# codyd51/gypsum

Measured on AMD Instinct MI355X. Metric: iq_msamples_per_s_32sat_acquire_plus_track, higher is better.
Workload: dtype f32; 1 GPU; cfg3 8.184Msps x128 streams/GPU: 32-sat acquire (13 scans/step) + 12-ch E-P-L track 1000ms/step; iq=resident in HBM (host-fed: legs.h2d), streams_per_gpu=128, satellites_searched=32, scene=SURVEY d2: a*N=41, sigma=6a (lock unreachable; lock-regime legs: *_lock), parallelism=streams sharded over 1 GPU(s), one ncclAllGather/step (gyp_allgather_dev)

## Files before the change

gypsum_amd/csrc/kernels_dll_exact.hpp:

```cpp
#pragma once
#include "kernels_track_block.hpp"

namespace gyp {

struct DllExactParams {
    const cf* iq;
    int64_t stream_stride;
    int32_t n_ms, ms_begin, ms_end;
    const double* start_time;
    const ChanState* states;
    int32_t n_chan;
    const SpecIn* spec;
    double* disc_out;
    const float* chipf;
    double inv_fs;
    const int32_t* only_if;
    const int32_t* from_sub;
    SubLayout sub;
    const int32_t* trk_round;
};

__device__ __forceinline__ double2 horner64(double2 acc, double2 w, double2 x) {
    return make_double2(fma(acc.x, w.x, fma(-acc.y, w.y, x.x)), fma(acc.x, w.y, fma(acc.y, w.x, x.y)));
}
__device__ __forceinline__ double2 cvt64(cf x) { return make_double2((double)x.x, (double)x.y); }
__device__ __forceinline__ double2 cvt64(double2 x) { return x; }
struct ExactChips { float cm1, c0, cp1; };
__device__ __forceinline__ ExactChips exact_window_chips(const float* chipf, int m, int q) {
    int j = m - q;
    j = j < 0 ? j + kChips : j;
    j = j < 0 ? j + kChips : j;
    const float* cp = chipf + j + kChips;
    return ExactChips{cp[-1], cp[0], cp[1]};
}
#pragma clang diagnostic push
#pragma clang diagnostic ignored "-Walign-mismatch"
typedef float4 __attribute__((aligned(8))) float4_a8;
__device__ __forceinline__ float4 load_pair_a8(const cf* src, int pair = 0) { return reinterpret_cast<const float4_a8*>(src)[pair]; }
#pragma clang diagnostic pop
template <int K, bool EDGE>
__device__ __forceinline__ ExactChips exact_window_load(const cf* __restrict__ block, int m, int r, int q, const float* __restrict__ chipf, cf (&x)[K]) {
    constexpr int N = K * kChips;
    const int n0 = K * m + r;
    if constexpr (EDGE) {
#pragma unroll
        for (int i = 0; i < K; ++i) {
            const int n = n0 + i;
            const cf v = block[min(max(n, 0), N - 1)];
            const bool in = n >= 0 && n < N;
            x[i] = make_float2(in ? v.x : 0.f, in ? v.y : 0.f);
        }
    } else {
        const cf* src = block + n0;
#pragma unroll
        for (int i = 0; i + 1 < K; i += 2) {
            const float4 v = load_pair_a8(src + i);
            x[i] = make_float2(v.x, v.y);
            x[i + 1] = make_float2(v.z, v.w);
        }
        if (K & 1) x[K - 1] = src[K - 1];
    }
    return exact_window_chips(chipf, m, q);
}
template <int K, typename S>
__device__ __forceinline__ void exact_window_fold(const S (&x)[K], const ExactChips& c, double2 rho, double2 step, double2& sp, double2& se, double2& sl) {
    const double dj = (double)c.c0, gl = (double)(c.cm1 - c.c0), ge = (double)(c.c0 - c.cp1);
    double2 h = cvt64(x[K - 1]);
#pragma unroll
    for (int i = K - 2; i >= 0; --i) h = horner64(h, rho, cvt64(x[i]));
    const double2 xe = cvt64(x[K - 1]), xl = cvt64(x[0]);
    sp = horner64(sp, step, make_double2(dj * h.x, dj * h.y));
    se = horner64(se, step, make_double2(ge * xe.x, ge * xe.y));
    sl = horner64(sl, step, make_double2(gl * xl.x, gl * xl.y));
}
template <int K, bool EDGE>
__device__ __forceinline__ void exact_window(const cf* __restrict__ block, int m, int r, int q, const float* __restrict__ chipf,
                                             double2 rho, double2 step, double2& sp, double2& se, double2& sl) {
    cf x[K];
    const ExactChips c = exact_window_load<K, EDGE>(block, m, r, q, chipf, x);
    exact_window_fold<K>(x, c, rho, step, sp, se, sl);
}
template <int K>
__device__ __forceinline__ double2 cpow_km1(double2 w) {
    double2 r = make_double2(1.0, 0.0);
#pragma unroll
    for (int i = 0; i < K - 1; ++i) r = cmul64(r, w);
    return r;
}
struct ExactUnit {
    double du, u0;
    int q, r;
    const float* chipf;
};
template <int K>
__device__ __forceinline__ ExactUnit exact_unit(const DllExactParams& p, const SpecIn& in, int sat, int ms) {
    ExactUnit u;
    u.chipf = p.chipf + (sat - 1) * 2048;
    u.du = in.doppler * p.inv_fs;
    u.u0 = carrier_cycles(in.doppler, p.start_time[ms], in.carrier_phase);
    const int sN = __builtin_amdgcn_readfirstlane(mod_n(in.code_phase, K * kChips));
    u.q = sN / K; u.r = sN % K;
    return u;
}
template <int K>
__device__ __forceinline__ void exact_unit_store(double2 sp, double2 se, double2 sl, const ExactUnit& u, int lane, int n_anchor, double* out) {
    const double2 rho_a = carrier64(u.du);
    const double2 anchor = carrier64(u.u0 + u.du * (double)n_anchor);
    const double2 pp = cmul64(sp, anchor), ee = cmul64(cmul64(se, cpow_km1<K>(rho_a)), anchor), ll = cmul64(sl, anchor);
    double acc[6] = {pp.x, pp.y, ee.x, ee.y, ll.x, ll.y};
#pragma unroll
    for (int v = 0; v < 6; ++v) acc[v] = wave_sum_last(acc[v]);
    if (lane == 63) *out = dll_discriminator_exact(acc);
}
__device__ __forceinline__ bool exact_unit_decode(const DllExactParams& p, int u, int& ch, int& ms) {
    if (!unit_decode(p, u, ch, ms)) return false;
    if (p.only_if && !p.only_if[ch]) return false;
    if (p.from_sub && ms < p.sub.begin(p.from_sub[ch])) return false;
    return true;
}
template <int K>
__global__ __launch_bounds__(256, 4) void dll_exact_wave_kernel(DllExactParams p) {
    static_assert(K <= 8, "a window's samples in registers");
    constexpr int N = K * kChips;
    const int lane = threadIdx.x & 63;
    const int wave = __builtin_amdgcn_readfirstlane((int)(threadIdx.x >> 6));
    const int n_units = p.n_chan * unit_span(p);
    const int n_groups = (n_units + 3) >> 2;
    for (int g = blockIdx.x; g < n_groups; g += gridDim.x) {
        const int u = ((n_groups & 7) ? g : xcd_contiguous(g, n_groups)) * 4 + wave;
        if (u >= n_units) continue;
        int ch, ms;
        if (!exact_unit_decode(p, u, ch, ms)) continue;
        const int64_t at = (int64_t)ch * p.n_ms + ms;
        const SpecIn in = p.spec[at];
        if (in.key == kSpecKeyLost) continue;
        const ChanState* st = p.states + ch;
        const int sat = __builtin_amdgcn_readfirstlane(st->sat_id), stream = __builtin_amdgcn_readfirstlane(st->stream);
        const cf* block = p.iq + (int64_t)stream * p.stream_stride + (int64_t)ms * N;
        const ExactUnit x = exact_unit<K>(p, in, sat, ms);
        double2 sp = make_double2(0.0, 0.0), se = sp, sl = sp;
        const double2 rho = carrier64(x.du), step = carrier64(x.du * (double)(K * 64));
        exact_window<K, true>(block, lane + 64 * 15 - 1, x.r, x.q, x.chipf, rho, step, sp, se, sl);
#pragma unroll 2
        for (int c = 14; c >= 1; --c) exact_window<K, false>(block, lane + 64 * c - 1, x.r, x.q, x.chipf, rho, step, sp, se, sl);
        exact_window<K, true>(block, lane - 1, x.r, x.q, x.chipf, rho, step, sp, se, sl);
        exact_unit_store<K>(sp, se, sl, x, lane, K * (lane - 1) + x.r, p.disc_out + at);
    }
}
constexpr int kExactSharedConsumers = 12;
constexpr int kExactSharedProducers = 4;
constexpr int kExactSharedThreads = 64 * (kExactSharedConsumers + kExactSharedProducers);
constexpr int kExactGroupMaxChan = 16384;
struct ExactGroup {
    int32_t stream, n;
    int32_t ch[kExactSharedConsumers];
    int32_t pad[2];
};
static_assert(sizeof(ExactGroup) == 64, "ExactGroup");
template <int K>
constexpr int exact_shared_lds_units() { return (K * kChips + 2 * K) / K * (K + 1); }
template <int K>
constexpr size_t exact_shared_lds_bytes() { return (size_t)exact_shared_lds_units<K>() * sizeof(double2); }

__global__ __launch_bounds__(256) void exact_group_kernel(const ChanState* __restrict__ states, int32_t n_chan, ExactGroup* __restrict__ groups,
                                                          int32_t* __restrict__ n_groups) {
    __shared__ int32_t s_stream[kExactGroupMaxChan];
    for (int i = threadIdx.x; i < n_chan; i += blockDim.x) s_stream[i] = states[i].stream;
    __syncthreads();
    const int c = blockIdx.x * blockDim.x + threadIdx.x;
    if (c >= n_chan) return;
    const int s = s_stream[c];
    int before = 0;
    for (int i = 0; i < c; ++i) before += s_stream[i] == s ? 1 : 0;
    if (before % kExactSharedConsumers) return;
    ExactGroup g;
    g.stream = s; g.n = 1; g.ch[0] = c; g.pad[0] = g.pad[1] = 0;
#pragma unroll
    for (int k = 1; k < kExactSharedConsumers; ++k) g.ch[k] = -1;
    for (int i = c + 1; i < n_chan && g.n < kExactSharedConsumers; ++i) {
        if (s_stream[i] != s) continue;
#pragma unroll
        for (int k = 1; k < kExactSharedConsumers; ++k)
            if (k == g.n) g.ch[k] = i;
        ++g.n;
    }
    groups[atomicAdd(n_groups, 1)] = g;
}

struct DllExactSharedParams {
    DllExactParams x;
    const ExactGroup* groups;
    const int32_t* n_groups;
};
template <int K>
__global__ __launch_bounds__(kExactSharedThreads) void dll_exact_shared_kernel(DllExactSharedParams ps) {
    static_assert(K <= 8, "a window's samples in registers");
    constexpr int N = K * kChips;
    static_assert(K % 2 == 0, "the producers fetch sample pairs");
    constexpr int PT = 64 * kExactSharedProducers;
    constexpr int PAIRS = N / 2;
    constexpr int LOADS = (PAIRS + PT - 1) / PT;
    extern __shared__ double2 s_x[];
    const DllExactParams& p = ps.x;
    const int lane = threadIdx.x & 63;
    const int wave = __builtin_amdgcn_readfirstlane((int)(threadIdx.x >> 6));
    const int span = p.ms_end - p.ms_begin;
    const int64_t n_items = (int64_t)__builtin_amdgcn_readfirstlane(ps.n_groups[0]) * span;
    const int64_t lo = n_items * blockIdx.x / gridDim.x, hi = n_items * (blockIdx.x + 1) / gridDim.x;
    if (lo >= hi) return;
    if (threadIdx.x < 2 * K) {
        const int np = threadIdx.x < K ? (int)threadIdx.x : N + (int)threadIdx.x;
        s_x[np + np / K] = make_double2(0.0, 0.0);
    }
    if (wave >= kExactSharedConsumers) {
        const int pt = lane + 64 * (wave - kExactSharedConsumers);
        float4 hold[LOADS];
        auto request = [&](int64_t item) {
            const int g = (int)(item / span), ms = p.ms_begin + (int)(item % span);
            const int stream = __builtin_amdgcn_readfirstlane(ps.groups[g].stream);
            const cf* block = p.iq + (int64_t)stream * p.stream_stride + (int64_t)ms * N;
#pragma unroll
            for (int j = 0; j < LOADS; ++j) {
                const int t = pt + PT * j;
                if (PT * j + PT <= PAIRS) hold[j] = load_pair_a8(block, t);
                else hold[j] = t < PAIRS ? load_pair_a8(block, t) : make_float4(0.f, 0.f, 0.f, 0.f);
            }
        };
        request(lo);
        for (int64_t item = lo; item < hi; ++item) {
#pragma unroll
            for (int j = 0; j < LOADS; ++j) {
                const int t = pt + PT * j, np = 2 * t + K;
                if (PT * j + PT <= PAIRS || t < PAIRS) {
                    s_x[np + np / K] = make_double2((double)hold[j].x, (double)hold[j].y);
                    s_x[np + np / K + 1] = make_double2((double)hold[j].z, (double)hold[j].w);
                }
            }
            __syncthreads();
            if (item + 1 < hi) request(item + 1);
            __syncthreads();
        }
        return;
    }
    const double2* win0 = s_x + (K + 1) * lane;
    for (int64_t item = lo; item < hi; ++item) {
        __syncthreads();
        const int g = (int)(item / span), ms = p.ms_begin + (int)(item % span);
        const ExactGroup* grp = ps.groups + g;
        const int ch = wave < __builtin_amdgcn_readfirstlane(grp->n) ? __builtin_amdgcn_readfirstlane(grp->ch[wave]) : -1;
        if (ch >= 0) {
            const int64_t at = (int64_t)ch * p.n_ms + ms;
            const SpecIn in = p.spec[at];
            if (in.key != kSpecKeyLost) {
                const ExactUnit u = exact_unit<K>(p, in, __builtin_amdgcn_readfirstlane(p.states[ch].sat_id), ms);
                int off[K];
#pragma unroll
                for (int i = 0; i < K; ++i) off[i] = u.r + i + (u.r + i >= K ? 1 : 0);
                double2 sp = make_double2(0.0, 0.0), se = sp, sl = sp;
                const double2 rho = carrier64(u.du), step = carrier64(u.du * (double)(K * 64));
#pragma unroll 2
                for (int c = 15; c >= 0; --c) {
                    const double2* w = win0 + (K + 1) * 64 * c;
                    double2 x[K];
#pragma unroll
                    for (int i = 0; i < K; ++i) x[i] = w[off[i]];
                    exact_window_fold<K>(x, exact_window_chips(u.chipf, lane + 64 * c - 1, u.q), rho, step, sp, se, sl);
                }
                exact_unit_store<K>(sp, se, sl, u, lane, K * (lane - 1) + u.r, p.disc_out + at);
            }
        }
        __syncthreads();
    }
}
template <int K, int T, int NV, bool PAIRS, bool GUARD, typename ParamsT, typename UseT>
__device__ __forceinline__ void workgroup_exact_sums(const cf* block, const ParamsT& p, const SpecIn& in, int ms, int lag,
                                                     const float* chipf, int tid, double (*part)[6], UseT use) {
    static_assert(!PAIRS || T == 256, "four wavefronts");
    const double du = in.doppler * p.inv_fs;
    const double u0 = carrier_cycles(in.doppler, p.start_time[ms], in.carrier_phase);
    double acc[6];
    exact_epl_generic<K, T>(block, u0, du, lag, chipf, tid, acc);
#pragma unroll
    for (int v = 0; v < NV; ++v) acc[v] = wave_sum_last(acc[v]);
    if (GUARD) __syncthreads();
    if ((tid & 63) == 63) {
#pragma unroll
        for (int v = 0; v < NV; ++v) part[tid >> 6][v] = acc[v];
    }
    __syncthreads();
    if (tid == 0) {
        double ex[NV];
#pragma unroll
        for (int v = 0; v < NV; ++v) {
            if (PAIRS) {
                ex[v] = (part[0][v] + part[1][v]) + (part[2][v] + part[3][v]);
            } else {
                double t = part[0][v];
#pragma unroll
                for (int w = 1; w < T / 64; ++w) t += part[w][v];
                ex[v] = t;
            }
        }
        use(ex);
    }
}
template <int K>
__global__ __launch_bounds__(256) void dll_exact_block_kernel(DllExactParams p) {
    constexpr int N = K * kChips;
    __shared__ double part[4][6];
    const int tid = threadIdx.x;
    const int n_units = p.n_chan * unit_span(p);
    for (int v = blockIdx.x; v < n_units; v += gridDim.x) {
        int ch, ms;
        if (!exact_unit_decode(p, (n_units & 7) ? v : xcd_contiguous(v, n_units), ch, ms)) continue;
        const int64_t at = (int64_t)ch * p.n_ms + ms;
        const SpecIn in = p.spec[at];
        if (in.key == kSpecKeyLost) continue;
        const ChanState* st = p.states + ch;
        const cf* block = p.iq + (int64_t)st->stream * p.stream_stride + (int64_t)ms * N;
        workgroup_exact_sums<K, 256, 6, true, true>(block, p, in, ms, mod_n(in.code_phase, N), p.chipf + (st->sat_id - 1) * 2048, tid, part,
                                                    [&](const double (&ex)[6]) { p.disc_out[at] = dll_discriminator_exact(ex); });
    }
}

struct DllScanParams {
    const cf* iq;
    int64_t stream_stride;
    int32_t n_ms, ms_begin, ms_end;
    const double* start_time;
    ChanState* states;
    const ChanState* ckpt;
    int32_t n_chan;
    const SpecIn* spec;
    const double* disc;
    gyp_track_rec* rec_out;
    DllExact* exact;
    const int32_t* bad;
    int32_t only_bad;
    const int32_t* from_sub;
    SubLayout sub;
    DllExact* hist_out;
    const float* chipf;
    double inv_fs, dll_gain, dll_modulus, n_samples;
    int32_t first, final;
    int32_t* prof_delta;
    int32_t prof_from, prof_depth;
    float symbol_tau;
    const int32_t* trk_round;
    DllExact* hist;
};
constexpr int kScanThreads = 256;
constexpr int kScanChunk = 512;
constexpr int kSpecKeyRepaired = -3;
__device__ __forceinline__ void scan_stage_code(float* s_chipf, const float* chipf, int tid) {
    for (int k = tid; k < 2048; k += kScanThreads) s_chipf[k] = chipf[k];
    __syncthreads();
}
template <int K>
__global__ __launch_bounds__(kScanThreads) void dll_scan_kernel(DllScanParams p) {
    constexpr int N = K * kChips;
    __shared__ double s_disc[kScanChunk];
    __shared__ int s_cpin[kScanChunk];
    __shared__ int s_cpout[kScanChunk];
    __shared__ int s_key[kScanChunk];
    __shared__ double part[kScanThreads / 64][6];
    __shared__ float s_chipf[2048];
    __shared__ double s_a;
    __shared__ int s_s, s_pos, s_repairs;
    __shared__ int s_nund;
    __shared__ short s_und[kScanChunk];
    bool have_code = false;
    const int ch = blockIdx.x, tid = threadIdx.x;
    if (ch >= p.n_chan) return;
    if (p.bad && (p.bad[ch] != 0) != (p.only_bad != 0)) return;
    const ChanState* st = p.states + ch;
    int range_lo = p.ms_begin, range_hi = p.ms_end, sub_here = -1;
    if (p.trk_round) {
        sub_here = p.trk_round[ch];
        if (sub_here < 0) return;
        range_lo = p.sub.begin(sub_here);
        range_hi = p.sub.end(sub_here, p.n_ms);
    }
    if (tid == 0) {
        if (p.trk_round) {
            if (sub_here == 0) { s_a = p.ckpt[ch].dll_phase; s_s = p.ckpt[ch].code_phase; s_repairs = 0; }
            else { const DllExact x = p.hist[(size_t)sub_here * p.n_chan + ch]; s_a = x.dll; s_s = x.code_phase; s_repairs = x.repairs; }
        } else if (p.first && p.ckpt) { s_a = p.ckpt[ch].dll_phase; s_s = p.ckpt[ch].code_phase; s_repairs = 0; }
        else { const DllExact x = p.exact[ch]; s_a = x.dll; s_s = x.code_phase; s_repairs = p.first ? 0 : x.repairs; }
    }
    const float* chipf = p.chipf + (st->sat_id - 1) * 2048;
    const cf* stream = p.iq + (int64_t)st->stream * p.stream_stride;
    const int64_t row = (int64_t)ch * p.n_ms;
    const int ms_first = (p.only_bad && p.from_sub) ? max(p.ms_begin, p.sub.begin(min(p.from_sub[ch], p.sub.sub_of(p.n_ms - 1)))) : range_lo;
    for (int c0 = ms_first; c0 < range_hi; c0 += kScanChunk) {
        const int len = min(kScanChunk, range_hi - c0);
        for (int i = tid; i < len; i += kScanThreads) {
            const SpecIn* in = p.spec + row + c0 + i;
            const int key = in->key;
            s_key[i] = key;
            s_cpin[i] = in->code_phase;
            s_disc[i] = key == kSpecKeyLost ? 0.0 : p.disc[row + c0 + i];
        }
        if (tid == 0) { s_pos = 0; s_nund = 0; }
        __syncthreads();
        if (p.rec_out) {
            for (int i = tid; i < len; i += kScanThreads) {
                const gyp_track_rec* r = p.rec_out + row + c0 + i;
                const float pr = r->peak_re, pi = r->peak_im;
                if (s_key[i] != kSpecKeyLost && r->status != 2 && fabsf(pr) <= p.symbol_tau * __builtin_amdgcn_sqrtf(fmaf(pr, pr, pi * pi)))
                    s_und[atomicAdd(&s_nund, 1)] = (short)i;
            }
            __syncthreads();
            const int n_und = s_nund;
            for (int u = 0; u < n_und; ++u) {
                const int ms = c0 + s_und[u];
                const SpecIn in = p.spec[row + ms];
                if (!have_code) { scan_stage_code(s_chipf, chipf, tid); have_code = true; }
                int lag = mod_n(in.code_phase, N) + p.rec_out[row + ms].peak_offset;
                lag = lag >= N ? lag - N : lag;
                workgroup_exact_sums<K, kScanThreads, 1, false, false>(
                    stream + (int64_t)ms * N, p, in, ms, lag, s_chipf, tid, part,
                    [&](const double (&re)[1]) { p.rec_out[row + ms].pseudosymbol = re[0] > 0.0 ? 1 : (re[0] < 0.0 ? -1 : 0); });
                __syncthreads();
            }
        }
        while (true) {
            if (tid < 64) {
                double a = s_a;
                int s = s_s, i = __builtin_amdgcn_readfirstlane(s_pos);
                bool stop = false;
                int key_n = 0, cp_n = 0;
                double d_n = 0.0;
                if (i < len) { key_n = s_key[i]; cp_n = s_cpin[i]; d_n = s_disc[i]; }
                while (i < len && !stop) {
                    const int key = key_n, cp = cp_n;
                    const double d = d_n;
                    if (i + 1 < len) { key_n = s_key[i + 1]; cp_n = s_cpin[i + 1]; d_n = s_disc[i + 1]; }
                    const double dll = __dadd_rn(a, __dmul_rn(d, p.dll_gain));
                    const double whole = trunc(dll);
                    const int usual = (int)(key != kSpecKeyLost) & ((int)(key == kSpecKeyRepaired) | (int)(s == cp)) &
                                      (int)(fabs(whole) < 2147483648.0) & (int)(dll > -p.dll_modulus) & (int)(dll < 2.0 * p.dll_modulus);
                    if (__builtin_amdgcn_readfirstlane(usual)) {
                        double r = dll >= p.dll_modulus ? dll - p.dll_modulus : dll;
                        r += (r != 0.0 && r < 0.0) ? p.dll_modulus : 0.0;
                        r += r < 0.0 ? p.dll_modulus : 0.0;
                        a = r;
                        s = (int)whole;
                        if (tid == 0) s_cpout[i] = s;
                        ++i;
                        continue;
                    }
                    if (uniform(key == kSpecKeyLost)) {
                        if (tid == 0) s_cpout[i] = s;
                        ++i;
                        continue;
                    }
                    if (uniform(key != kSpecKeyRepaired && s != cp)) { stop = true; break; }
                    double r = pymod_uniform(dll, p.dll_modulus);
                    r += r < 0.0 ? p.dll_modulus : 0.0;
                    a = r;
                    s = uniform(fabs(whole) < 2147483648.0) ? (int)whole : code_phase_beyond_int32(whole, p.n_samples);
                    if (tid == 0) s_cpout[i] = s;
                    ++i;
                }
                if (tid == 0) { s_a = a; s_s = s; s_pos = i; }
            }
            __syncthreads();
            const int pos = s_pos;
            if (pos >= len) break;
            {
                const int ms = c0 + pos;
                const SpecIn in = p.spec[row + ms];
                if (!have_code) { scan_stage_code(s_chipf, chipf, tid); have_code = true; }
                workgroup_exact_sums<K, kScanThreads, 6, false, false>(stream + (int64_t)ms * N, p, in, ms, mod_n(s_s, N), s_chipf, tid, part, [&](const double (&ex)[6]) {
                    s_disc[pos] = dll_discriminator_exact(ex);
                    s_key[pos] = kSpecKeyRepaired;
                    if (p.rec_out) {
                        gyp_track_rec* rec = p.rec_out + row + ms;
                        int lag = rec->peak_offset + mod_n(in.code_phase, N);
                        lag = lag >= N ? lag - N : lag;
                        const int k2 = lag - mod_n(s_s, N);
                        rec->peak_offset = k2 < 0 ? k2 + N : k2;
                    }
                    if (p.prof_delta && ms >= p.prof_from)
                        p.prof_delta[(int64_t)ch * p.prof_depth + (ms - p.prof_from)] = mod_n(s_s, N) - mod_n(in.code_phase, N);
                    ++s_repairs;
                });
                __syncthreads();
            }
        }
        if (p.rec_out) {
            for (int i = tid; i < len; i += kScanThreads) {
                gyp_track_rec* rec = p.rec_out + row + c0 + i;
                rec->code_phase = s_cpout[i];
                if (s_key[i] != kSpecKeyLost) rec->discriminator = (float)s_disc[i];
            }
        }
        __syncthreads();
    }
    if (tid == 0) {
        DllExact x; x.dll = s_a; x.code_phase = s_s; x.repairs = s_repairs;
        if (p.trk_round) {
            p.hist[(size_t)(sub_here + 1) * p.n_chan + ch] = x;
        } else {
            p.exact[ch] = x;
            if (p.hist_out) p.hist_out[ch] = x;
            if (p.final) { p.states[ch].dll_phase = s_a; p.states[ch].code_phase = s_s; }
        }
    }
}

}
```

Baseline: 11650 Msamples/s.

## Cache chip coefficients as bitmasks and specialize shared DLL windows per residue

```diff
diff --git a/gypsum_amd/csrc/kernels_dll_exact.hpp b/gypsum_amd/csrc/kernels_dll_exact.hpp
--- a/gypsum_amd/csrc/kernels_dll_exact.hpp
+++ b/gypsum_amd/csrc/kernels_dll_exact.hpp
@@ -63,8 +63,7 @@
     return exact_window_chips(chipf, m, q);
 }
 template <int K, typename S>
-__device__ __forceinline__ void exact_window_fold(const S (&x)[K], const ExactChips& c, double2 rho, double2 step, double2& sp, double2& se, double2& sl) {
-    const double dj = (double)c.c0, gl = (double)(c.cm1 - c.c0), ge = (double)(c.c0 - c.cp1);
+__device__ __forceinline__ void exact_window_fold_coef(const S (&x)[K], double dj, double ge, double gl, double2 rho, double2 step, double2& sp, double2& se, double2& sl) {
     double2 h = cvt64(x[K - 1]);
 #pragma unroll
     for (int i = K - 2; i >= 0; --i) h = horner64(h, rho, cvt64(x[i]));
@@ -72,6 +71,10 @@
     sp = horner64(sp, step, make_double2(dj * h.x, dj * h.y));
     se = horner64(se, step, make_double2(ge * xe.x, ge * xe.y));
     sl = horner64(sl, step, make_double2(gl * xl.x, gl * xl.y));
+}
+template <int K, typename S>
+__device__ __forceinline__ void exact_window_fold(const S (&x)[K], const ExactChips& c, double2 rho, double2 step, double2& sp, double2& se, double2& sl) {
+    exact_window_fold_coef<K>(x, (double)c.c0, (double)(c.c0 - c.cp1), (double)(c.cm1 - c.c0), rho, step, sp, se, sl);
 }
 template <int K, bool EDGE>
 __device__ __forceinline__ void exact_window(const cf* __restrict__ block, int m, int r, int q, const float* __restrict__ chipf,
@@ -102,6 +105,21 @@
     u.q = sN / K; u.r = sN % K;
     return u;
 }
+template <int CTRL>
+__device__ __forceinline__ double dpp_d_any(double v) {
+    const unsigned lo = __builtin_amdgcn_mov_dpp((unsigned)__double2loint(v), CTRL, 0xF, 0xF, true);
+    const unsigned hi = __builtin_amdgcn_mov_dpp((unsigned)__double2hiint(v), CTRL, 0xF, 0xF, true);
+    return __hiloint2double((int)hi, (int)lo);
+}
+__device__ __forceinline__ double wave_sum_lane63(double v) {
+    v += dpp_d_any<kDppXor1>(v);
+    v += dpp_d_any<kDppXor2>(v);
+    v += dpp_d_any<kDppHalfMirror>(v);
+    v += dpp_d_any<kDppMirror>(v);
+    v += dpp_d_any<0x142>(v);
+    v += dpp_d_any<0x143>(v);
+    return v;
+}
 template <int K>
 __device__ __forceinline__ void exact_unit_store(double2 sp, double2 se, double2 sl, const ExactUnit& u, int lane, int n_anchor, double* out) {
     const double2 rho_a = carrier64(u.du);
@@ -109,7 +127,7 @@
     const double2 pp = cmul64(sp, anchor), ee = cmul64(cmul64(se, cpow_km1<K>(rho_a)), anchor), ll = cmul64(sl, anchor);
     double acc[6] = {pp.x, pp.y, ee.x, ee.y, ll.x, ll.y};
 #pragma unroll
-    for (int v = 0; v < 6; ++v) acc[v] = wave_sum_last(acc[v]);
+    for (int v = 0; v < 6; ++v) acc[v] = wave_sum_lane63(acc[v]);
     if (lane == 63) *out = dll_discriminator_exact(acc);
 }
 __device__ __forceinline__ bool exact_unit_decode(const DllExactParams& p, int u, int& ch, int& ms) {
@@ -192,6 +210,52 @@
     const ExactGroup* groups;
     const int32_t* n_groups;
 };
+struct ExactCoefBits {
+    uint32_t dj;
+    uint32_t ge, gl;
+};
+__device__ __forceinline__ ExactCoefBits exact_coef_bits(const float* __restrict__ chipf, int lane, int q) {
+    ExactCoefBits b{0u, 0u, 0u};
+#pragma unroll
+    for (int c = 0; c < 16; ++c) {
+        const ExactChips k = exact_window_chips(chipf, lane + 64 * c - 1, q);
+        const uint32_t m = __float_as_uint(k.cm1) >> 31, z = __float_as_uint(k.c0) >> 31, n = __float_as_uint(k.cp1) >> 31;
+        b.dj |= z << c;
+        b.ge |= ((z ^ n) | ((z & ~n) << 1)) << (2 * c);
+        b.gl |= ((m ^ z) | ((m & ~z) << 1)) << (2 * c);
+    }
+    return b;
+}
+typedef double __attribute__((ext_vector_type(2))) lds_d2;
+typedef const __attribute__((address_space(3))) lds_d2* lds_d2_ptr;
+template <int K, int R>
+__device__ __forceinline__ void exact_shared_windows(uint32_t lds_win0, const ExactCoefBits& b, double2 rho, double2 step, double2& sp, double2& se, double2& sl) {
+    int z0 = 0, z1 = 0, z2 = 0;
+    asm volatile("" : "+v"(z0), "+v"(z1), "+v"(z2));
+#pragma unroll 2
+    for (int c = 15; c >= 0; --c) {
+        uint32_t at = lds_win0 + (uint32_t)sizeof(double2) * (K + 1) * 64 * c;
+        asm volatile("" : "+v"(at));
+        const lds_d2_ptr w = (lds_d2_ptr)at;
+        double2 x[K];
+#pragma unroll
+        for (int i = 0; i < K; ++i) {
+            const lds_d2 v = w[R + i + (R + i >= K ? 1 : 0)];
+            x[i] = make_double2(v.x, v.y);
+        }
+        const double dj = __hiloint2double((int)(((b.dj << (31 - c)) & 0x80000000u) | 0x3FF00000u), z0);
+        const double ge = __hiloint2double((int)((b.ge << (30 - 2 * c)) & 0xC0000000u), z1);
+        const double gl = __hiloint2double((int)((b.gl << (30 - 2 * c)) & 0xC0000000u), z2);
+        exact_window_fold_coef<K>(x, dj, ge, gl, rho, step, sp, se, sl);
+    }
+}
+template <int K, int R = 0>
+__device__ __forceinline__ void exact_shared_windows_at(int r, uint32_t lds_win0, const ExactCoefBits& b, double2 rho, double2 step, double2& sp, double2& se, double2& sl) {
+    if constexpr (R + 1 < K) {
+        if (r != R) { exact_shared_windows_at<K, R + 1>(r, lds_win0, b, rho, step, sp, se, sl); return; }
+    }
+    exact_shared_windows<K, R>(lds_win0, b, rho, step, sp, se, sl);
+}
 template <int K>
 __global__ __launch_bounds__(kExactSharedThreads) void dll_exact_shared_kernel(DllExactSharedParams ps) {
     static_assert(K <= 8, "a window's samples in registers");
@@ -242,7 +306,9 @@
         }
         return;
     }
-    const double2* win0 = s_x + (K + 1) * lane;
+    const uint32_t lds_win0 = (uint32_t)(uintptr_t)(const __attribute__((address_space(3))) double2*)s_x + (uint32_t)sizeof(double2) * (K + 1) * lane;
+    ExactCoefBits bits{0u, 0u, 0u};
+    int have_ch = -1, have_sat = 0, have_q = 0;
     for (int64_t item = lo; item < hi; ++item) {
         __syncthreads();
         const int g = (int)(item / span), ms = p.ms_begin + (int)(item % span);
@@ -252,20 +318,15 @@
             const int64_t at = (int64_t)ch * p.n_ms + ms;
             const SpecIn in = p.spec[at];
             if (in.key != kSpecKeyLost) {
-                const ExactUnit u = exact_unit<K>(p, in, __builtin_amdgcn_readfirstlane(p.states[ch].sat_id), ms);
-                int off[K];
-#pragma unroll
-                for (int i = 0; i < K; ++i) off[i] = u.r + i + (u.r + i >= K ? 1 : 0);
+                const int sat = __builtin_amdgcn_readfirstlane(p.states[ch].sat_id);
+                const ExactUnit u = exact_unit<K>(p, in, sat, ms);
+                if (ch != have_ch || sat != have_sat || u.q != have_q) {
+                    bits = exact_coef_bits(u.chipf, lane, u.q);
+                    have_ch = ch; have_sat = sat; have_q = u.q;
+                }
                 double2 sp = make_double2(0.0, 0.0), se = sp, sl = sp;
                 const double2 rho = carrier64(u.du), step = carrier64(u.du * (double)(K * 64));
-#pragma unroll 2
-                for (int c = 15; c >= 0; --c) {
-                    const double2* w = win0 + (K + 1) * 64 * c;
-                    double2 x[K];
-#pragma unroll
-                    for (int i = 0; i < K; ++i) x[i] = w[off[i]];
-                    exact_window_fold<K>(x, exact_window_chips(u.chipf, lane + 64 * c - 1, u.q), rho, step, sp, se, sl);
-                }
+                exact_shared_windows_at<K>(u.r, lds_win0, bits, rho, step, sp, se, sl);
                 exact_unit_store<K>(sp, se, sl, u, lane, K * (lane - 1) + u.r, p.disc_out + at);
             }
         }
```

After: 11750 Msamples/s (median of 6 runs). About the same (+0.9%).
